# matthieugomez/LeastSquaresOptim.jl

Hardware: AMD Instinct MI355X
Metric: lm_lsmr_outer_iterations_per_sec (higher is better)
Workload: dtype f64

## Files before the change

leastsquaresoptim.jl_amd/csrc/lsq_lsmr.hip:

```cpp
#include <chrono>
#include <cmath>
#include <cstdlib>

#include "lsq_solver.h"
#include "lsq_spmv.h"

static constexpr int LSQ_LOOKAHEAD_DEFAULT = 2;

__device__ __forceinline__ void publish(LsqMailbox *mail, const LsmrState *st) {
    unsigned long long w = ((unsigned long long)(st->epoch & 0x7fffffu) << 41) |
                           ((unsigned long long)(st->done ? 1 : 0) << 40) |
                           ((unsigned long long)(st->istop & 0xff) << 32) | (unsigned)st->iter;
    __hip_atomic_store((unsigned long long *)mail, w, __ATOMIC_RELEASE, __HIP_MEMORY_SCOPE_SYSTEM);
}

__global__ void __launch_bounds__(LSQ_NT)
k_lsmr_prep(int n, const double *__restrict__ colsum, double *__restrict__ damp, double *__restrict__ P,
            double *__restrict__ dg, double *__restrict__ ux, int custom_p) {
    for (int j = blockIdx.x * LSQ_NT + threadIdx.x; j < n; j += gridDim.x * LSQ_NT) {
        double s = colsum[j];
        if (damp) {
            double d = damp[j];
            s += d;
            double r = sqrt(d);
// ... 335 lines not shown
#pragma unroll
    for (int k = 0; k < R; ++k) {
        const int i = tid + k * 1024;
        if (i < n) {
            acc += cs[k];
            double gi = gv[k];
            if (lm.lo && lm.x[i] <= lm.lo[i] && gi > 0.0) gi = 0.0;
            else if (lm.hi && lm.x[i] >= lm.hi[i] && gi < 0.0) gi = 0.0;
            double a = fabs(gi);
            if (isnan(a)) a = INFINITY;
            mg = fmax(mg, a);
        }
    }
    acc = wave_sum(acc);
    mg = wave_max(mg);
    if ((tid & 63) == 0) {
        sh[tid >> 6] = acc;
        shm[tid >> 6] = mg;
    }
    __syncthreads();
    if (tid == 0) {
        double tt = 0.0, tm = shm[0];
        for (int w = 0; w < 16; ++w) tt += sh[w];
        for (int w = 1; w < 16; ++w) tm = fmax(tm, shm[w]);
        s_mean = tt / n;
        if (blockIdx.x == 0) {
            *lm.out_grad = tm;
            st->iter = 0; st->istop = 0; st->done = 0; st->notdone = 1; st->first = 1;
            st->atol = atol; st->btol = btol; st->ctol = ctol;
            st->maxiter = maxiter; st->epoch = epoch; st->cu = 0.0;
            pu[0] = ysumsq;
            *npu = 1;
        }
    }
    __syncthreads();
    const double lo_d = lm.min_diag * s_mean, hi_d = lm.max_diag * s_mean;
    const double beta = dampened_norm(ysumsq, 0.0);
    const bool beta_zero = !(beta > 0.0);
    const double inv_beta = beta > 0.0 ? 1.0 / beta : 1.0;
    double a2 = 0.0;
    const int j = blockIdx.x * 1024 + tid;
    if (j < n) {
        double c0 = 0.0, g0 = 0.0;
#pragma unroll
        for (int k = 0; k < R; ++k)
            if (k == (int)blockIdx.x) { c0 = cs[k]; g0 = gv[k]; }
        double c = c0;
        c = c > hi_d ? hi_d : (c < lo_d ? lo_d : c);
        const double d = c * lm.inv_delta;
        const double s = c0 + d;
        const double r = sqrt(d);
        dg[j] = r;
        damp[j] = r;
        ux[j] = 0.0;
        const double Pj = s > 0.0 ? 1.0 / sqrt(s) : 0.0;
        P[j] = Pj;
        if (!beta_zero) {
            const double w = g0 * inv_beta * Pj;
            v[j] = w;
            if (wout) wout[j] = colscale ? (w * Pj) * colscale[j] : w * Pj;
            a2 = w * w;
        }
    }
    __syncthreads();
    const double bv = block_sum<1024>(a2, sh);
    if (tid == 0) {
        pv[blockIdx.x] = bv;
        if (blockIdx.x == 0) *npv = (int)gridDim.x;
    }
}

struct EpiBuf {
    static constexpr bool REDUCE = false;
    const int *done;
    int extra_blocks;
    double *out;
    double *partials;
    unsigned *counter;
    __device__ void seg(int j, double dot, double &) const { out[j] = dot; }
    __device__ void extra(int, double &) const {}
    __device__ void finalize(double) const {}
};
__global__ void __launch_bounds__(LSQ_NT) k_rowshard_sumsq(const double *pu, const int *npu, double *out, const int *done,
                                                            double *xbuf, int n) {
    if (done && *done) {
        for (int i = threadIdx.x; i <= n; i += LSQ_NT) xbuf[i] = 0.0;
        return;
    }
    double a, b, c2;
    ordered_sum256x3(pu, npu, nullptr, nullptr, nullptr, nullptr, a, b, c2);
    if (threadIdx.x == 0) *out = a;
}
extern "C" int lsq_solver_set_row_allreduce(lsq_solver *s, lsq_device_allreduce_callback cb, void *user, long long global_rows) {
    if (!s || s->kind != LSQ_LSMR) {
        lsq_set_error("row-sharded solves: LSMR() only");
        return LSQ_EARG;
    }
    s->row_cb = cb;
    s->row_user = user;
    s->global_rows = cb ? global_rows : 0;
    s->colsum_g_uid = 0;
    s->colsum_g_version = ~0ull;
    if (cb && !s->d_xbuf) {
        LSQ_HIP(hipMalloc(&s->d_xbuf, (size_t)(s->n + 2 + 256) * sizeof(double)));
        LSQ_ZERO(s->d_xbuf, 0, (size_t)(s->n + 2 + 256) * sizeof(double));
        LSQ_HIP(hipMalloc(&s->d_one, sizeof(int)));
        const int one = 1;
        LSQ_HIP(hipMemcpy(s->d_one, &one, sizeof(int), hipMemcpyHostToDevice));
    }
    return LSQ_OK;
}
int lsq_rowshard_colsum(lsq_solver *s, lsq_mat *J, const double **out) {
    const double *local = lsq_cached_colsum(J);
    if (!local) return LSQ_EHIP;
    *out = local;
    if (!s->row_cb) return LSQ_OK;
    lsq_ctx *c = s->ctx;
    if (!s->d_colsum_g) LSQ_HIP(hipMalloc(&s->d_colsum_g, (size_t)(s->n > 0 ? s->n : 1) * sizeof(double)));
    if (s->colsum_g_uid != J->uid || s->colsum_g_version != J->version) {
        LSQ_TRY(lsq_d2d(c, s->d_colsum_g, local, (size_t)J->n * sizeof(double)));
        if (s->row_cb(s->d_colsum_g, J->n, (void *)c->stream, s->row_user) != 0) {
            lsq_set_error("row all-reduce callback reported failure");
            return LSQ_ECALLBACK;
        }
        s->colsum_g_uid = J->uid;
        s->colsum_g_version = J->version;
    }
    *out = s->d_colsum_g;
    return LSQ_OK;
}
static int rowshard_adjoint(lsq_solver *s, lsq_mat *J, const double *src, EpiV ev, const double *pu, const int *npu) {
    lsq_ctx *c = s->ctx;
    const int n = J->n;
    EpiBuf eb{ev.done, 0, s->d_xbuf, nullptr, nullptr};
    LSQ_TRY(launch_product(J, 1, src, eb));
    LSQ_LAUNCH(k_rowshard_sumsq, dim3(1), dim3(LSQ_NT), 0, c->stream, pu, npu, s->d_xbuf + n, ev.done, s->d_xbuf, n);
    LSQ_HIP(hipGetLastError());
    if (s->row_cb(s->d_xbuf, n + 1, (void *)c->stream, s->row_user) != 0) {
        lsq_set_error("row all-reduce callback reported failure");
        return LSQ_ECALLBACK;
    }
    ev.pu = s->d_xbuf + n;
    ev.npu = s->d_one;
    const int nb = lsq_div_up(n, LSQ_CMB_COLS);
    LSQ_LAUNCH((k_combine<EpiV>), dim3(std::min(nb, 2048)), dim3(LSQ_NT), 0, c->stream, s->d_xbuf, n, 1, ev, nb);
    LSQ_HIP(hipGetLastError());
    return LSQ_OK;
}

int lsq_lsmr_alloc(lsq_solver *s) {
    size_t nb = (size_t)(s->n > 0 ? s->n : 1) * sizeof(double);
    LSQ_HIP(hipMalloc(&s->d_state, 2 * sizeof(LsmrState)));
    LSQ_ZERO(s->d_state, 0, 2 * sizeof(LsmrState));
    s->f3_elems = 4 * (size_t)(s->n > 0 ? s->n : 1) + 2 * 4096 + 8 + 16 + 8;
    LSQ_HIP(hipMalloc(&s->d_f3, s->f3_elems * sizeof(double)));
    LSQ_ZERO(s->d_f3, 0, s->f3_elems * sizeof(double));
    LSQ_HIP(hipMalloc(&s->d_u, (size_t)(s->m > 0 ? s->m : 1) * sizeof(double)));
    LSQ_HIP(hipMalloc(&s->d_ux, nb));
    LSQ_HIP(hipMalloc(&s->d_v, nb));
    LSQ_HIP(hipMalloc(&s->d_h, nb));
    LSQ_HIP(hipMalloc(&s->d_hbar, nb));
    LSQ_HIP(hipMalloc(&s->d_t, nb));
    LSQ_HIP(hipMalloc(&s->d_P, nb));
    LSQ_HIP(hipMalloc(&s->d_dg, nb));
    LSQ_HIP(hipMalloc(&s->d_rhs, nb));
    LSQ_HIP(hipMalloc(&s->d_red, 4 * 4096 * sizeof(double) + 64));
    LSQ_ZERO(s->d_red, 0, 4 * 4096 * sizeof(double) + 64);
    return LSQ_OK;
}

void lsq_lsmr_free(lsq_solver *s) {
    hipFree(s->d_state); hipFree(s->d_u); hipFree(s->d_ux); hipFree(s->d_v); hipFree(s->d_h);
    hipFree(s->d_hbar); hipFree(s->d_t); hipFree(s->d_P); hipFree(s->d_dg); hipFree(s->d_rhs); hipFree(s->d_red);
    hipFree(s->d_xbuf); hipFree(s->d_one); hipFree(s->d_colsum_g); hipFree(s->d_f3);
}

static inline int nvec_grid(const lsq_ctx *c, int n) {
    int g = lsq_div_up(n > 0 ? n : 1, LSQ_NT);
    int cap = c->num_cus * 4;
    return g > cap ? cap : g;
}

bool lsq_lsmr_takes_lm_prep(const lsq_solver *s, const lsq_mat *J) {
    return s->kind == LSQ_LSMR && J->n <= LSMR_LM_PREP_MAX_N && (s->row_cb || !lsq_small_mat(J)) && !s->precond_cb && !s->gen_ldiv &&
           !getenv("LSQ_LSMR_SEPARATE_SETUP");
}

struct LsmrProgress {
    bool ours, done;
    int istop, iter;
    LsmrProgress(unsigned long long w, unsigned epoch)
        : ours((unsigned)(w >> 41) == epoch), done(((w >> 40) & 1ull) != 0), istop((int)((w >> 32) & 0xff)), iter((int)(w & 0xffffffffu)) {}
};
static inline unsigned long long lsmr_progress_word(const lsq_ctx *c) { return *(volatile unsigned long long *)c->h_mail; }

struct StopPredictor {
    double t1_prev, t2_prev, ratio2;
    int hint_it;
    int update(const LsqMailbox *mail, unsigned long long w, int it, double atol, double btol) {
        if (!(it > hint_it && it >= 1)) return 0;
        const double h1 = mail->test1, h2 = mail->test2;
        const unsigned long long w2 = *(volatile unsigned long long *)mail;
        if (!(w2 == w && h1 > 0.0 && h2 > 0.0)) return 0;
        if (t2_prev > 0.0 && h2 < t2_prev) ratio2 = std::min(0.95, std::max(1e-4, h2 / t2_prev));
        int k = 1 << 20;
        if (h2 > atol && ratio2 < 1.0) k = std::min(k, (int)std::ceil(std::log(atol / h2) / std::log(ratio2) - 1e-9));
        if (t1_prev > 0.0 && h1 < 0.98 * t1_prev && h1 > btol)
            k = std::min(k, (int)std::ceil(std::log(btol / h1) / std::log(h1 / t1_prev) - 1e-9));
        t1_prev = h1; t2_prev = h2; hint_it = it;
        return k < (1 << 20) ? it + std::max(1, k) : 0;
    }
};

struct LsmrRun {
    int it = 0, istop = 0;
    bool finished = false;
    bool tail_ran = false;
    bool see(const LsmrProgress &p) {
        if (p.ours) it = p.iter;
        if (p.ours && p.done) { istop = p.istop; finished = true; }
        return finished;
    }
};

static int lsmr_stream_drained(lsq_ctx *c, unsigned epoch, int committed, const LsmrState *d_st, bool spent, LsmrRun &r) {
    const hipError_t sq = hipStreamQuery(c->stream);
    if (sq != hipSuccess && sq != hipErrorNotReady) {
        lsq_set_error("HIP error inside the LSMR iteration: %s", hipGetErrorString(sq));
        return LSQ_EHIP;
    }
    if (sq != hipSuccess) return LSQ_OK;
    const LsmrProgress p(lsmr_progress_word(c), epoch);
    if (p.ours && (p.done || p.iter >= committed)) return LSQ_OK;
    LsmrState hs;
    LSQ_HIP(hipMemcpy(&hs, d_st, sizeof(hs), hipMemcpyDeviceToHost));
    r.it = hs.iter;
    if (hs.done) {
        r.istop = hs.istop;
        r.finished = true;
    } else if (spent) {
        lsq_set_error("lsmr: iteration budget exhausted without a stop rule");
        return LSQ_EHIP;
    }
    return LSQ_OK;
}

struct LsmrProf {
    size_t base[2];
    std::vector<int> iter[2];
};
static void lsmr_drop_idle_samples(lsq_ctx *c, LsmrProf &p, int it) {
    for (int k = 0; k < 2; ++k) {
        auto &v = c->prof_ev[k];
        while (v.size() > p.base[k] && !p.iter[k].empty() && p.iter[k].back() > it) {
            hipEventDestroy(v.back()); v.pop_back();
            hipEventDestroy(v.back()); v.pop_back();
            p.iter[k].pop_back();
        }
    }
}

struct LsmrWork {
    lsq_solver *s;
    lsq_ctx *c;
    lsq_mat *J;
    const double *d_y;
    double *d_x;
    int m, n;
    bool damped, sharded;
    bool fused;
    double atol, btol, conlim;
    int maxiter, lookahead;
    unsigned epoch;
    int gn;
    const double *dgk;
    const LsmrTail *tail;
    bool dynamic, spec;
    LsmrState *stb[2];
    double *pu, *pv;
    int *npu, *npv;
    double *pxb[2];
    int *npxb[2];
    double *vset;
    double *fx[2], *fhbar[2], *fh[2];
    double *fw;
    double *fpu[2];
    int *fnpu;
    LsmrHandoff *fho;
};

static EpiV lsmr_epi_v(const LsmrWork &W) {
    return EpiV{&W.stb[0]->done, 0, W.stb[0], W.pu, W.npu, nullptr, nullptr, W.s->d_P, W.dgk, nullptr, W.s->d_v, W.pv, W.npv,
                nullptr, 0.0, 0.0, 0, 0};
}
static void lsmr_launch_update(const LsmrWork &W, bool summed, const double *px_in, const int *npx_in, int out) {
    lsq_solver *s = W.s; lsq_ctx *c = W.c;
    LSQ_LAUNCH(k_lsmr_update, dim3(W.gn), dim3(LSQ_NT), 0, c->stream, W.n, W.stb[0], c->d_mail,
                       summed ? (const double *)(s->d_xbuf + W.n) : (const double *)W.pu,
                       summed ? (const int *)s->d_one : (const int *)W.npu, W.pv, W.npv, px_in, npx_in, W.pxb[out], W.npxb[out],
                       W.dgk, s->d_ux, s->d_P, s->d_v, s->d_h, s->d_hbar, s->d_rhs, W.d_x, s->d_t, c->d_partials, lsq_ctr(c, 3));
}

static int lsmr_enqueue_setup(const LsmrWork &W, double *d_damp, const double *d_Jty, double y_sumsq, const LsmrLmPrep *lm,
                              const double *colsum, int custom_p) {
    lsq_solver *s = W.s; lsq_ctx *c = W.c; lsq_mat *J = W.J;
    const int m = W.m, n = W.n;
    LsmrState *st = W.stb[0];
// ... 122 lines not shown
        }
        if (!(wait_at > 0 && r.it < wait_at)) {
            if (k1 == enq + 1) {
                LSQ_TRY(launch_k2());
                spins = 0;
                continue;
            }
            if (enq - r.it < W.lookahead + 1 && enq < W.maxiter + 1) {
                const bool guess = W.spec && planned > 0 && enq >= planned && enq >= 1;
                const bool unknown = W.spec && enq == 1 && pred.hint_it == 0 && tail->predict <= 3;
                LSQ_TRY(launch_k1(guess || unknown));
                if (guess || unknown) {
                    wait_at = enq;
                    wait_is_guess = guess;
                }
                spins = 0;
                continue;
            }
        }
        if (c->idle_hook) lsq_run_idle_hook(c);
        if ((++spins & 0x3ffu) != 0) continue;
        LSQ_TRY(lsmr_stream_drained(c, W.epoch, k1 - 1, W.stb[k1 & 1], enq >= W.maxiter + 1, r));
    }
    lsmr_drop_idle_samples(c, prof, r.it);
    if (r.istop == 99) {
        lsq_set_error("lsmr: the in-launch hand-off of k_lsmr_fused timed out");
        return LSQ_EHIP;
    }
    if (wait_at > 0 && wait_is_guess) c->tail_spec[0]++;
    return LSQ_OK;
}

static int lsmr_run_four(const LsmrWork &W, StopPredictor &pred, LsmrRun &r) {
    lsq_solver *s = W.s; lsq_ctx *c = W.c; lsq_mat *J = W.J;
    const LsmrTail *tail = W.tail;
    const bool sharded = W.sharded;
    const int maxiter = W.maxiter;
    LsmrState *st = W.stb[0];
    EpiU eu{&st->done, 0, st, W.d_y, s->d_u, W.n, s->d_dg, s->d_t, s->d_ux, W.pu, W.npu, nullptr, 0.0};
    EpiV ev = lsmr_epi_v(W);
    ev.ux = W.damped ? s->d_ux : nullptr;
    int planned = W.spec ? tail->predict : 0;
    int tail_at = 0;
    int enq = 0;
    LsmrProf prof{{c->prof_ev[0].size(), c->prof_ev[1].size()}, {}};
    unsigned long long spins = 0;
    while (!r.finished) {
        const unsigned long long w = lsmr_progress_word(c);
        const LsmrProgress p(w, W.epoch);
        if (r.see(p)) break;
        if (W.spec && p.ours && tail_at > 0 && r.it >= tail_at) {
            c->tail_spec[0]++;
            c->tail_spec[1]++;
            tail_at = 0;
            planned = 0;
        }
        if (W.dynamic && p.ours) {
            const int stop = pred.update(c->h_mail, w, r.it, W.atol, W.btol);
            if (stop > 0 && tail_at == 0) planned = stop;
        }
        if (W.spec && tail_at == 0 && planned > 0 && enq >= planned && enq > r.it) {
            LSQ_TRY(tail->fn(&st->notdone, tail->user));
            tail_at = enq;
        }
        const bool hold = tail_at > 0 && enq == tail_at && r.it < tail_at;
        const bool want = sharded ? (p.ours && enq == r.it && enq < maxiter) : (!hold && enq - r.it < W.lookahead && enq < maxiter);
        if (want) {
            const int chunk = sharded ? (int)std::min<long long>(W.lookahead, (long long)maxiter - enq) : 1;
            for (int q = 0; q < chunk; ++q) {
                if (c->prof_kernels & 1) lsq_prof_mark(c, 0, 0);
                {
                    const size_t before = c->prof_ev[0].size();
                    LSQ_TRY(launch_product(J, 0, s->d_t, eu));
                    if (c->prof_ev[0].size() > before) prof.iter[0].push_back(enq + 1);
                }
                if (c->prof_kernels & 1) lsq_prof_mark(c, 0, 1);
                eu.uold = s->d_u;
                const int cur = enq & 1;
                ev.px = W.damped ? W.pxb[cur] : nullptr;
                ev.npx = W.npxb[cur];
                if (c->prof_kernels & 2) lsq_prof_mark(c, 1, 0);
                {
                    const size_t before = c->prof_ev[1].size();
                    if (sharded) LSQ_TRY(rowshard_adjoint(s, J, s->d_u, ev, W.pu, W.npu));
                    else LSQ_TRY(launch_product(J, 1, s->d_u, ev));
                    if (c->prof_ev[1].size() > before) prof.iter[1].push_back(enq + 1);
                }
                if (c->prof_kernels & 2) lsq_prof_mark(c, 1, 1);
                lsmr_launch_update(W, sharded, ev.px, ev.npx, cur ^ 1);
                LSQ_HIP(hipGetLastError());
                ++enq;
            }
            spins = 0;
            continue;
        }
        if (c->idle_hook) lsq_run_idle_hook(c);
        if ((++spins & 0x3ffu) != 0) continue;
        LSQ_TRY(lsmr_stream_drained(c, W.epoch, enq, st, enq >= maxiter, r));
    }
    lsmr_drop_idle_samples(c, prof, r.it);
    if (tail_at > 0) {
        c->tail_spec[0]++;
        if (r.it > tail_at) c->tail_spec[1]++;
        else r.tail_ran = true;
    }
    return LSQ_OK;
}

int lsq_lsmr_solve(lsq_solver *s, lsq_mat *J, const double *d_y, double *d_damp, double *d_x, int *nmul,
                   const double *d_Jty, double y_sumsq, const LsmrLmPrep *lm, const LsmrTail *tail) {
    lsq_ctx *c = s->ctx;
    const int m = J->m, n = J->n;
    if (m != s->m || n != s->n) {
        lsq_set_error("lsmr: solver allocated for %dx%d, Jacobian is %dx%d", s->m, s->n, m, n);
        return LSQ_EDIM;
    }
    if (s->gen_ldiv) {
        if (s->row_cb) {
            lsq_set_error("row-sharded solves take diagonal preconditioners only");
            return LSQ_EARG;
        }
        LSQ_TRY(lsq_lsmr_general_solve(s, J, d_y, d_damp, d_x, nmul));
        s->last_lsmr_path = 4;
        return tail && tail->fn ? tail->fn(nullptr, tail->user) : LSQ_OK;
    }
    const bool sharded = s->row_cb != nullptr;
    if (lsq_small_mat(J) && !s->precond_cb && !sharded) {
        LSQ_TRY(lsq_lsmr_exact_solve(s, J, d_y, d_damp, d_x, nmul));
        s->last_lsmr_path = 1;
        return tail && tail->fn ? tail->fn(nullptr, tail->user) : LSQ_OK;
    }
    LsmrWork W;
    W.s = s; W.c = c; W.J = J; W.d_y = d_y; W.d_x = d_x; W.m = m; W.n = n;
    W.damped = d_damp != nullptr; W.sharded = sharded;
    W.atol = 1e-6; W.btol = W.damped ? 0.5 : 1e-6; W.conlim = 1e8;
    const long long rows = (sharded ? s->global_rows : (long long)m) + (W.damped ? n : 0);
    W.maxiter = (int)std::max<long long>(rows, n);
    W.lookahead = lsq_dbg_serial ? 1 : LSQ_LOOKAHEAD_DEFAULT;
    W.epoch = (++c->mail_epoch) & 0x7fffffu;
    if (J->kind == LSQ_MAT_CSC) LSQ_TRY(lsq_ensure_csr(J));
    const bool four_env = getenv("LSQ_LSMR_FOUR_LAUNCHES") != nullptr;
    W.fused = !four_env && !sharded && J->kind == LSQ_MAT_CSC && J->srows.active && J->srows.ncw == 1 && J->scols.active &&
              n >= 1 && m >= 1 && c->num_cus >= 8;
    W.gn = nvec_grid(c, n); W.dgk = W.damped ? s->d_dg : nullptr;
    W.tail = tail;
    W.dynamic = tail && tail->fn && tail->dynamic && !sharded;
    W.spec = tail && tail->fn && !sharded && (tail->predict > 0 || W.dynamic);
    W.stb[0] = s->d_state; W.stb[1] = s->d_state + 1;
    W.pv = s->d_red + 4096;
    W.pxb[0] = s->d_red + 2 * 4096; W.pxb[1] = s->d_red + 3 * 4096;
    int *const counts = (int *)(s->d_red + 4 * 4096);
    W.npv = counts + 1; W.npxb[0] = counts + 2; W.npxb[1] = counts + 3;
    double *const f3 = s->d_f3;
    W.fx[0] = s->d_rhs; W.fx[1] = f3; W.fhbar[0] = s->d_hbar; W.fhbar[1] = f3 + n; W.fh[0] = s->d_h; W.fh[1] = f3 + 2 * (size_t)n;
    W.fw = f3 + 3 * (size_t)n;
    W.fpu[0] = f3 + 4 * (size_t)n; W.fpu[1] = W.fpu[0] + 4096;
    W.fnpu = (int *)(W.fpu[1] + 4096); W.fho = (LsmrHandoff *)(W.fpu[1] + 4096 + 8);
    W.vset = W.fused ? s->d_t : s->d_v;
    W.pu = W.fused ? W.fpu[0] : s->d_red;
    W.npu = W.fused ? W.fnpu : counts;
    const double *colsum = nullptr;
    LSQ_TRY(lsq_rowshard_colsum(s, J, &colsum));
    const int custom_p = s->precond_cb ? 1 : 0;
    if (custom_p) {
        LSQ_HIP(hipStreamSynchronize(c->stream));
        if (s->precond_cb(s->d_P, J, d_damp, s->precond_user) != 0) {
            lsq_set_error("preconditioner callback reported failure");
            return LSQ_ECALLBACK;
        }
    }
    *(volatile unsigned long long *)c->h_mail = 0ull;
    LSQ_TRY(lsmr_enqueue_setup(W, d_damp, d_Jty, y_sumsq, lm, colsum, custom_p));

    StopPredictor pred{-1.0, -1.0, s->lsmr_ratio2, 0};
    LsmrRun r;
    LSQ_TRY(W.fused ? lsmr_run_fused(W, pred, r) : lsmr_run_four(W, pred, r));
    s->last_iter = r.it;
    s->last_istop = r.istop;
    s->last_lsmr_path = W.fused ? 3 : 2;
    if (nmul) *nmul = 2 * r.it;
    if (W.dynamic && pred.t2_prev > 0.0) s->lsmr_ratio2 = pred.ratio2;
    if (tail && tail->fn && !r.tail_ran) LSQ_TRY(tail->fn(nullptr, tail->user));
    return LSQ_OK;
}
```

leastsquaresoptim.jl_amd/csrc/lsq_lsmr3.h:

```cpp
#pragma once

constexpr int LSQ_FUSED_UB_MAX = 4;
struct LsmrHandoff {
    unsigned long long w[8];
};
__device__ __forceinline__ void lsmr_handoff_write(LsmrHandoff *ho, unsigned tag, double vs, double cu, int done) {
    const unsigned long long t = (unsigned long long)tag << 32;
    const unsigned long long bv = (unsigned long long)__double_as_longlong(vs), bc = (unsigned long long)__double_as_longlong(cu);
    __hip_atomic_store(&ho->w[0], t | (bv & 0xffffffffull), __ATOMIC_RELAXED, __HIP_MEMORY_SCOPE_AGENT);
    __hip_atomic_store(&ho->w[1], t | (bv >> 32), __ATOMIC_RELAXED, __HIP_MEMORY_SCOPE_AGENT);
    __hip_atomic_store(&ho->w[2], t | (bc & 0xffffffffull), __ATOMIC_RELAXED, __HIP_MEMORY_SCOPE_AGENT);
    __hip_atomic_store(&ho->w[3], t | (bc >> 32), __ATOMIC_RELAXED, __HIP_MEMORY_SCOPE_AGENT);
    __hip_atomic_store(&ho->w[4], t | (unsigned)done, __ATOMIC_RELAXED, __HIP_MEMORY_SCOPE_AGENT);
}
__device__ __forceinline__ void lsmr_handoff_fail(LsmrHandoff *ho, unsigned tag) {
    __hip_atomic_store(&ho->w[6], (unsigned long long)tag, __ATOMIC_RELAXED, __HIP_MEMORY_SCOPE_AGENT);
}
struct LsmrHandoffWords { unsigned long long w[5]; };
__device__ __forceinline__ LsmrHandoffWords lsmr_handoff_request(const LsmrHandoff *ho) {
    LsmrHandoffWords r;
#pragma unroll
    for (int k = 0; k < 5; ++k) r.w[k] = __hip_atomic_load(&ho->w[k], __ATOMIC_RELAXED, __HIP_MEMORY_SCOPE_AGENT);
    return r;
}
__device__ __forceinline__ bool lsmr_handoff_valid(const LsmrHandoffWords &r, unsigned tag) {
    bool ok = true;
#pragma unroll
    for (int k = 0; k < 5; ++k) ok = ok && (unsigned)(r.w[k] >> 32) == tag;
    return ok;
}
struct LsmrFused {
    const LsmrState *st_in;
    LsmrState *st_out;
    LsqMailbox *mail;
    LsmrHandoff *ho;
    unsigned tag;
    unsigned tag_prev;
    const double *pu_in; const int *npu_in;
    double *pu_out; int *npu_out;
    const double *px_in; const int *npx_in;
    double *px_out; int *npx_out;
    const double *pv; const int *npv;
    const double *vt;
    const double *w;
    const double *P, *dg;
    const double *h_in, *hbar_in, *x_in;
    double *h_out, *hbar_out, *x_out;
    double *v, *xout, *ux;
    const double *uold; double *unew;
    int n, ub;
    int test_no_record;
    int cautious;
};

__device__ inline void lsmr_decide(LsmrState &s, double total) {
    s.iter += 1;
    s.normx = sqrt(total);
    const double test1 = s.normr / s.normb;
    const double test2 = s.normAr / (s.normA * s.normr);
    const double test3 = 1.0 / s.condA;
    const double t1 = test1 / (1.0 + s.normA * s.normx / s.normb);
    const double rtol = s.btol + s.atol * s.normA * s.normx / s.normb;
    int istop = 0;
    if (s.iter >= s.maxiter) istop = 7;
    else if (1.0 + test3 <= 1.0) istop = 6;
    else if (1.0 + test2 <= 1.0) istop = 5;
    else if (1.0 + t1 <= 1.0) istop = 4;
    else if (test3 <= s.ctol) istop = 3;
    else if (test2 <= s.atol) istop = 2;
    else if (test1 <= rtol) istop = 1;
    s.istop = istop;
    if (istop) { s.done = 1; s.notdone = 0; }
}

constexpr long long LSQ_FUSED_SPIN_LIMIT = 1LL << 24;

__device__ __forceinline__ void publish_relaxed(LsqMailbox *mail, const LsmrState *st) {
    unsigned long long w = ((unsigned long long)(st->epoch & 0x7fffffu) << 41) |
                           ((unsigned long long)(st->done ? 1 : 0) << 40) |
                           ((unsigned long long)(st->istop & 0xff) << 32) | (unsigned)st->iter;
    __hip_atomic_store((unsigned long long *)mail, w, __ATOMIC_RELAXED, __HIP_MEMORY_SCOPE_SYSTEM);
}

__device__ __forceinline__ void ordered_sum512x3(const double *pa, const int *na, const double *pb, const int *nb,
                                                 const double *pc, const int *nc, double &ra, double &rb, double &rc) {
    __shared__ double s_w5[3][4];
    __shared__ double s_tot5[3];
    const int tid = threadIdx.x;
    if (tid < 256) {
        const double a0 = pa ? pa[tid] : 0.0, b0 = pb ? pb[tid] : 0.0, c0 = pc ? pc[tid] : 0.0;
        const double a1 = pa ? pa[tid + 256] : 0.0, b1 = pb ? pb[tid + 256] : 0.0, c1 = pc ? pc[tid + 256] : 0.0;
        const int ca = pa ? *na : 0, cb = pb ? *nb : 0, cc = pc ? *nc : 0;
        double a = tid < ca ? a0 : 0.0, b = tid < cb ? b0 : 0.0, c = tid < cc ? c0 : 0.0;
        if (tid + 256 < ca) a += a1;
        if (tid + 256 < cb) b += b1;
        if (tid + 256 < cc) c += c1;
        for (int i = tid + 512; i < ca; i += 256) a += pa[i];
        for (int i = tid + 512; i < cb; i += 256) b += pb[i];
        for (int i = tid + 512; i < cc; i += 256) c += pc[i];
        a = wave_sum(a);
        b = wave_sum(b);
        c = wave_sum(c);
        if ((tid & 63) == 0) {
            s_w5[0][tid >> 6] = a;
            s_w5[1][tid >> 6] = b;
            s_w5[2][tid >> 6] = c;
        }
    }
    __syncthreads();
    if (tid < 3) s_tot5[tid] = ((s_w5[tid][0] + s_w5[tid][1]) + s_w5[tid][2]) + s_w5[tid][3];
    __syncthreads();
    ra = s_tot5[0];
    rb = s_tot5[1];
    rc = s_tot5[2];
    __syncthreads();
}

__device__ __forceinline__ void lsq_lds_barrier() { asm volatile("s_waitcnt lgkmcnt(0)\n\ts_barrier" ::: "memory"); }
template <bool IS_MAX>
__device__ __forceinline__ double lsq_block_reduce_lds(double v, double *sh ) {
    v = IS_MAX ? wave_max(v) : wave_sum(v);
    const int lane = threadIdx.x & 63, w = threadIdx.x >> 6;
    if (lane == 0) sh[w] = v;
    lsq_lds_barrier();
    double r = 0.0;
    if (threadIdx.x == 0) {
        r = sh[0];
#pragma unroll
        for (int i = 1; i < LSQ_BIG_NT / 64; ++i) r = IS_MAX ? fmax(r, sh[i]) : r + sh[i];
    }
    lsq_lds_barrier();
    return r;
}

template <int = 0>
__global__ void __launch_bounds__(LSQ_BIG_NT) k_lsmr_fused(SellDev S, int wrows, int m, int nxpad, LsmrFused a) {
    extern __shared__ __attribute__((aligned(16))) double smem[];
    __shared__ double sh[LSQ_BIG_NT / 64];
    __shared__ LsmrState ns;
    __shared__ double s_vs, s_cu;
    __shared__ int s_done;
    double *xl = smem;
    double *yw = smem + nxpad;
    const int tid = threadIdx.x, lane = tid & 63, wv = tid >> 6;
    const int n = a.n;
    const bool upd = (int)blockIdx.x < a.ub;

    if (upd) {
        static_assert(sizeof(LsmrState) % 8 == 0 && sizeof(LsmrState) / 8 <= LSQ_BIG_NT, "state copy: one 8-byte word per thread");
        constexpr int NQ = (LSQ_LDS_X_MAX + LSQ_BIG_NT - 1) / LSQ_BIG_NT;
        double xi[NQ], hbi[NQ], hi[NQ];
#pragma unroll
        for (int q = 0; q < NQ; ++q) {
            const int j = min(tid + q * LSQ_BIG_NT, n - 1);
            xi[q] = a.x_in[j];
            hbi[q] = a.hbar_in[j];
            hi[q] = a.h_in[j];
        }
        if (tid < (int)(sizeof(LsmrState) / 8)) ((unsigned long long *)&ns)[tid] = ((const unsigned long long *)a.st_in)[tid];
        const bool prev_failed = a.tag_prev != 0u &&
                                 (unsigned)__hip_atomic_load(&a.ho->w[6], __ATOMIC_RELAXED, __HIP_MEMORY_SCOPE_AGENT) == a.tag_prev;
        double beta2, betax2, alpha2;
        ordered_sum512x3(a.pu_in, a.npu_in, a.px_in, a.npx_in, a.pv, a.npv, beta2, betax2, alpha2);
        if (ns.done) {
            if (blockIdx.x == 0) {
                if (tid < (int)(sizeof(LsmrState) / 8)) ((unsigned long long *)a.st_out)[tid] = ((const unsigned long long *)&ns)[tid];
                if (tid == 0) {
                    lsmr_handoff_write(a.ho, a.tag, 1.0, 0.0, 1);
                    publish_relaxed(a.mail, &ns);
                }
            }
            return;
        }
        const bool was_first = ns.first != 0;
        if (tid == 0) lsmr_scalars(ns, beta2, betax2, alpha2, a.dg != nullptr, a.px_in != nullptr);
        __syncthreads();
        if (!was_first) {
            const double c1 = ns.c1, c2 = ns.c2;
            double acc = 0.0;
#pragma unroll
            for (int q = 0; q < NQ; ++q) {
                const double hb = hbi[q] * c1 + hi[q];
                const double xj = xi[q] + c2 * hb;
                acc += (tid + q * LSQ_BIG_NT < n) ? xj * xj : 0.0;
            }
            const double total = block_sum<LSQ_BIG_NT>(acc, sh);
            if (tid == 0) lsmr_decide(ns, total);
        } else if (tid == 0) {
            ns.first = 0;
            if (!(ns.normAr != 0.0)) { ns.done = 1; ns.notdone = 0; }
        }
        if (tid == 0 && prev_failed) { ns.istop = 99; ns.done = 1; ns.notdone = 0; }
        __syncthreads();
        const bool done_now = ns.done != 0;
        const double vs = ns.vscale, cu = ns.cu, c1 = ns.c1, c2 = ns.c2, c3 = ns.c3;
        if (blockIdx.x == 0) {
            if (tid == 0 && !a.test_no_record) lsmr_handoff_write(a.ho, a.tag, vs, cu, done_now ? 1 : 0);
            if (tid < (int)(sizeof(LsmrState) / 8)) ((unsigned long long *)a.st_out)[tid] = ((const unsigned long long *)&ns)[tid];
            if (tid == 0) {
                if (!was_first) {
                    __hip_atomic_store((double *)&a.mail->test1, ns.normr / ns.normb, __ATOMIC_RELAXED, __HIP_MEMORY_SCOPE_SYSTEM);
                    __hip_atomic_store((double *)&a.mail->test2, ns.normAr / (ns.normA * ns.normr), __ATOMIC_RELAXED, __HIP_MEMORY_SCOPE_SYSTEM);
                }
                publish_relaxed(a.mail, &ns);
            }
        }
        constexpr int NU = (NQ + 2) / 3;
        double e_vt[NU], e_P[NU], e_dg[NU], e_ux[NU], e_h[NU], e_hb[NU], e_x[NU];
#pragma unroll
        for (int k = 0; k < NU; ++k) {
            const int j = min((int)(blockIdx.x + k * a.ub) * LSQ_BIG_NT + tid, n - 1);
            e_vt[k] = a.vt[j];
            e_P[k] = a.P ? a.P[j] : 1.0;
            e_dg[k] = a.dg ? a.dg[j] : 0.0;
            e_ux[k] = a.dg ? a.ux[j] : 0.0;
            e_h[k] = a.h_in[j];
            e_hb[k] = a.hbar_in[j];
            e_x[k] = a.x_in[j];
        }
        double aux = 0.0;
#pragma unroll
        for (int k = 0; k < NU; ++k) {
            const int j = (int)(blockIdx.x + k * a.ub) * LSQ_BIG_NT + tid;
            if (j >= n) continue;
            const double Pj = e_P[k];
            const double vj = e_vt[k] * vs;
            a.v[j] = vj;
            if (was_first) {
                a.h_out[j] = vj;
                a.hbar_out[j] = 0.0;
                a.x_out[j] = 0.0;
                a.xout[j] = 0.0;
            } else {
                const double hj = e_h[k];
                const double hb = e_hb[k] * c1 + hj;
                a.hbar_out[j] = hb;
                const double xj = e_x[k] + c2 * hb;
                a.x_out[j] = xj;
                a.h_out[j] = hj * c3 + vj;
                a.xout[j] = a.P ? xj * Pj : xj;
            }
            if (a.dg && !done_now) {
                const double tj = a.P ? vj * Pj : vj;
                const double un = tj * e_dg[k] - cu * e_ux[k];
                a.ux[j] = un;
                aux += un * un;
            }
        }
        if (done_now) return;
        const double bux = lsq_block_reduce_lds<false>(aux, sh);
        if (tid == 0) {
            a.px_out[blockIdx.x] = bux;
            if (blockIdx.x == 0) *a.npx_out = a.ub;
        }
        return;
    }

    constexpr int XR = (LSQ_LDS_X_MAX + LSQ_BIG_NT - 1) / LSQ_BIG_NT;
    {
        double xr[XR];
#pragma unroll
        for (int q = 0; q < XR; ++q) xr[q] = a.w[min(tid + q * LSQ_BIG_NT, n - 1)];
        const int dflag = a.st_in->done;
#pragma unroll
        for (int q = 0; q < XR; ++q)
            if (tid + q * LSQ_BIG_NT < n) xl[tid + q * LSQ_BIG_NT] = xr[q];
        if (dflag) return;
    }
    constexpr int Q = LSQ_SELL_ROWS_MAX / LSQ_BIG_NT;
    const int pb = (int)blockIdx.x - a.ub, npb = (int)gridDim.x - a.ub;
    double racc = 0.0;
    bool have_scalars = false;
    if (a.cautious) {
        if (tid == 0) {
            LsmrHandoffWords rec = lsmr_handoff_request(a.ho);
            long long spins = 0;
            while (!lsmr_handoff_valid(rec, a.tag)) {
                if (++spins > (a.test_no_record ? 4096 : LSQ_FUSED_SPIN_LIMIT)) break;
                __builtin_amdgcn_s_sleep(8);
                rec = lsmr_handoff_request(a.ho);
            }
            const bool ok = spins <= (a.test_no_record ? 4096 : LSQ_FUSED_SPIN_LIMIT);
            s_vs = __longlong_as_double((long long)((rec.w[0] & 0xffffffffull) | (rec.w[1] << 32)));
            s_cu = __longlong_as_double((long long)((rec.w[2] & 0xffffffffull) | (rec.w[3] << 32)));
            s_done = ok ? (int)(rec.w[4] & 0xffffffffull) : 2;
            if (!ok) lsmr_handoff_fail(a.ho, a.tag);
        }
        __syncthreads();
        if (s_done) return;
        have_scalars = true;
    }
    for (int w = pb; w < S.nblocks; w += npb) {
        const int base = w * wrows, rows = min(wrows, m - base);
        const int s0 = w * S.spw, s1 = s0 + S.spw;
        double pre[Q];
#pragma unroll
        for (int q = 0; q < Q; ++q) pre[q] = a.uold[base + min(tid + q * LSQ_BIG_NT, rows - 1)];
        LsmrHandoffWords rec;
#pragma unroll
        for (int k = 0; k < 5; ++k) rec.w[k] = 0ull;
        {
            constexpr int NW = LSQ_BIG_NT / 64;
            int sidx = s0 + wv;
            SellSliceRef A = sell_slice_ref(S, sidx, s1, lane);
            __syncthreads();
            unsigned long long poll = 0ull;
            for (; sidx < s1; sidx += NW) {
                if (!have_scalars && (unsigned)(poll >> 32) == a.tag && (poll & 1ull)) break;
                if (!have_scalars) poll = __hip_atomic_load(&a.ho->w[4], __ATOMIC_RELAXED, __HIP_MEMORY_SCOPE_AGENT);
                const SellSliceRef r = A;
                A = sell_slice_ref(S, sidx + NW, s1, lane);
                if (!have_scalars && tid == 0 && sidx + NW >= s1) rec = lsmr_handoff_request(a.ho);
                const size_t oa = (size_t)r.sm.x + lane * 2;
                const unsigned pos = r.inf & LSQ_SELL_POS_MASK;
                double sum = 0.0, sq = 0.0;
                sell_lane_sum<false>(S.val + oa, S.idx16 + oa, r.sm.y, (int)(r.inf >> LSQ_SELL_POS_BITS), xl, sum, sq, lane);
                if (pos != LSQ_SELL_POS_MASK) yw[pos] = sum;
            }
        }
        if (!have_scalars && tid == 0) {
            long long spins = 0;
            while (!lsmr_handoff_valid(rec, a.tag)) {
                if (++spins > (a.test_no_record ? 4096 : LSQ_FUSED_SPIN_LIMIT)) break;
                __builtin_amdgcn_s_sleep(8);
                rec = lsmr_handoff_request(a.ho);
            }
            const bool ok = spins <= (a.test_no_record ? 4096 : LSQ_FUSED_SPIN_LIMIT);
            s_vs = __longlong_as_double((long long)((rec.w[0] & 0xffffffffull) | (rec.w[1] << 32)));
            s_cu = __longlong_as_double((long long)((rec.w[2] & 0xffffffffull) | (rec.w[3] << 32)));
            s_done = ok ? (int)(rec.w[4] & 0xffffffffull) : 2;
            if (!ok) lsmr_handoff_fail(a.ho, a.tag);
        }
        have_scalars = true;
        __syncthreads();
        if (s_done) return;
        const double vs = s_vs, cu = s_cu;
#pragma unroll
        for (int q = 0; q < Q; ++q) {
            const int i = tid + q * LSQ_BIG_NT;
            if (i < rows) {
                const double un = vs * yw[i] - cu * pre[q];
                a.unew[base + i] = un;
                racc += un * un;
            }
        }
    }
    const double bv = block_sum<LSQ_BIG_NT>(racc, sh);
    if (tid == 0) {
        a.pu_out[pb] = bv;
        if (pb == 0) *a.npu_out = npb;
    }
}
```

Measured before the change: 4210.

## Stage fused LSMR kernel vectors into LDS via async DMA and prefetch first slice

After: 4201. Within noise of the previous version (-0.2%).

```diff
diff --git a/leastsquaresoptim.jl_amd/csrc/lsq_lsmr.hip b/leastsquaresoptim.jl_amd/csrc/lsq_lsmr.hip
--- a/leastsquaresoptim.jl_amd/csrc/lsq_lsmr.hip
+++ b/leastsquaresoptim.jl_amd/csrc/lsq_lsmr.hip
@@ -511,7 +511,7 @@
     size_t nb = (size_t)(s->n > 0 ? s->n : 1) * sizeof(double);
     LSQ_HIP(hipMalloc(&s->d_state, 2 * sizeof(LsmrState)));
     LSQ_ZERO(s->d_state, 0, 2 * sizeof(LsmrState));
-    s->f3_elems = 4 * (size_t)(s->n > 0 ? s->n : 1) + 2 * 4096 + 8 + 16 + 8;
+    s->f3_elems = 4 * (((size_t)(s->n > 0 ? s->n : 1) + 1) & ~(size_t)1) + 2 * 4096 + 8 + 16 + 8;
     LSQ_HIP(hipMalloc(&s->d_f3, s->f3_elems * sizeof(double)));
     LSQ_ZERO(s->d_f3, 0, s->f3_elems * sizeof(double));
     LSQ_HIP(hipMalloc(&s->d_u, (size_t)(s->m > 0 ? s->m : 1) * sizeof(double)));
@@ -940,9 +940,10 @@
     int *const counts = (int *)(s->d_red + 4 * 4096);
     W.npv = counts + 1; W.npxb[0] = counts + 2; W.npxb[1] = counts + 3;
     double *const f3 = s->d_f3;
-    W.fx[0] = s->d_rhs; W.fx[1] = f3; W.fhbar[0] = s->d_hbar; W.fhbar[1] = f3 + n; W.fh[0] = s->d_h; W.fh[1] = f3 + 2 * (size_t)n;
-    W.fw = f3 + 3 * (size_t)n;
-    W.fpu[0] = f3 + 4 * (size_t)n; W.fpu[1] = W.fpu[0] + 4096;
+    const size_t np2 = ((size_t)n + 1) & ~(size_t)1;
+    W.fx[0] = s->d_rhs; W.fx[1] = f3; W.fhbar[0] = s->d_hbar; W.fhbar[1] = f3 + np2; W.fh[0] = s->d_h; W.fh[1] = f3 + 2 * np2;
+    W.fw = f3 + 3 * np2;
+    W.fpu[0] = f3 + 4 * np2; W.fpu[1] = W.fpu[0] + 4096;
     W.fnpu = (int *)(W.fpu[1] + 4096); W.fho = (LsmrHandoff *)(W.fpu[1] + 4096 + 8);
     W.vset = W.fused ? s->d_t : s->d_v;
     W.pu = W.fused ? W.fpu[0] : s->d_red;
diff --git a/leastsquaresoptim.jl_amd/csrc/lsq_lsmr3.h b/leastsquaresoptim.jl_amd/csrc/lsq_lsmr3.h
--- a/leastsquaresoptim.jl_amd/csrc/lsq_lsmr3.h
+++ b/leastsquaresoptim.jl_amd/csrc/lsq_lsmr3.h
@@ -149,19 +149,31 @@
     if (upd) {
         static_assert(sizeof(LsmrState) % 8 == 0 && sizeof(LsmrState) / 8 <= LSQ_BIG_NT, "state copy: one 8-byte word per thread");
         constexpr int NQ = (LSQ_LDS_X_MAX + LSQ_BIG_NT - 1) / LSQ_BIG_NT;
-        double xi[NQ], hbi[NQ], hi[NQ];
+        constexpr int NU = (NQ + 2) / 3;
+        const SellStageTail xtail = sell_stage_dma<(NQ + 1) / 2>(a.x_in, smem, n, tid);
+        double hbi[NQ], hi[NQ];
 #pragma unroll
         for (int q = 0; q < NQ; ++q) {
             const int j = min(tid + q * LSQ_BIG_NT, n - 1);
-            xi[q] = a.x_in[j];
             hbi[q] = a.hbar_in[j];
             hi[q] = a.h_in[j];
+        }
+        double e_vt[NU], e_P[NU], e_dg[NU], e_ux[NU];
+#pragma unroll
+        for (int k = 0; k < NU; ++k) {
+            const int j = min((int)(blockIdx.x + k * a.ub) * LSQ_BIG_NT + tid, n - 1);
+            e_vt[k] = a.vt[j];
+            e_P[k] = a.P ? a.P[j] : 1.0;
+            e_dg[k] = a.dg ? a.dg[j] : 0.0;
+            e_ux[k] = a.dg ? a.ux[j] : 0.0;
         }
         if (tid < (int)(sizeof(LsmrState) / 8)) ((unsigned long long *)&ns)[tid] = ((const unsigned long long *)a.st_in)[tid];
         const bool prev_failed = a.tag_prev != 0u &&
                                  (unsigned)__hip_atomic_load(&a.ho->w[6], __ATOMIC_RELAXED, __HIP_MEMORY_SCOPE_AGENT) == a.tag_prev;
         double beta2, betax2, alpha2;
         ordered_sum512x3(a.pu_in, a.npu_in, a.px_in, a.npx_in, a.pv, a.npv, beta2, betax2, alpha2);
+        sell_stage_tail_write(xtail, smem);
+        sell_stage_wait();
         if (ns.done) {
             if (blockIdx.x == 0) {
                 if (tid < (int)(sizeof(LsmrState) / 8)) ((unsigned long long *)a.st_out)[tid] = ((const unsigned long long *)&ns)[tid];
@@ -173,7 +185,22 @@
             return;
         }
         const bool was_first = ns.first != 0;
-        if (tid == 0) lsmr_scalars(ns, beta2, betax2, alpha2, a.dg != nullptr, a.px_in != nullptr);
+        if (wv == 0) {
+            double *park = smem + nxpad + lane;
+#pragma unroll
+            for (int q = 0; q < NQ; ++q) {
+                park[(2 * q) * 64] = hbi[q];
+                park[(2 * q + 1) * 64] = hi[q];
+            }
+            asm volatile("" ::: "memory");
+            if (tid == 0) lsmr_scalars(ns, beta2, betax2, alpha2, a.dg != nullptr, a.px_in != nullptr);
+            asm volatile("" ::: "memory");
+#pragma unroll
+            for (int q = 0; q < NQ; ++q) {
+                hbi[q] = park[(2 * q) * 64];
+                hi[q] = park[(2 * q + 1) * 64];
+            }
+        }
         __syncthreads();
         if (!was_first) {
             const double c1 = ns.c1, c2 = ns.c2;
@@ -181,7 +208,7 @@
 #pragma unroll
             for (int q = 0; q < NQ; ++q) {
                 const double hb = hbi[q] * c1 + hi[q];
-                const double xj = xi[q] + c2 * hb;
+                const double xj = smem[min(tid + q * LSQ_BIG_NT, n - 1)] + c2 * hb;
                 acc += (tid + q * LSQ_BIG_NT < n) ? xj * xj : 0.0;
             }
             const double total = block_sum<LSQ_BIG_NT>(acc, sh);
@@ -205,24 +232,22 @@
                 publish_relaxed(a.mail, &ns);
             }
         }
-        constexpr int NU = (NQ + 2) / 3;
-        double e_vt[NU], e_P[NU], e_dg[NU], e_ux[NU], e_h[NU], e_hb[NU], e_x[NU];
+        double aux = 0.0;
+        int ubs = a.ub, bxs = (int)blockIdx.x;
+        asm volatile("" : "+s"(ubs), "+s"(bxs));
 #pragma unroll
         for (int k = 0; k < NU; ++k) {
-            const int j = min((int)(blockIdx.x + k * a.ub) * LSQ_BIG_NT + tid, n - 1);
-            e_vt[k] = a.vt[j];
-            e_P[k] = a.P ? a.P[j] : 1.0;
-            e_dg[k] = a.dg ? a.dg[j] : 0.0;
-            e_ux[k] = a.dg ? a.ux[j] : 0.0;
-            e_h[k] = a.h_in[j];
-            e_hb[k] = a.hbar_in[j];
-            e_x[k] = a.x_in[j];
-        }
-        double aux = 0.0;
-#pragma unroll
-        for (int k = 0; k < NU; ++k) {
-            const int j = (int)(blockIdx.x + k * a.ub) * LSQ_BIG_NT + tid;
+            const int g = bxs + k * ubs;
+            const int j = g * LSQ_BIG_NT + tid;
             if (j >= n) continue;
+            double e_h = 0.0, e_hb = 0.0;
+#pragma unroll
+            for (int q = 0; q < NQ; ++q)
+                if (q == g) {
+                    e_h = hi[q];
+                    e_hb = hbi[q];
+                }
+            const double e_x = smem[j];
             const double Pj = e_P[k];
             const double vj = e_vt[k] * vs;
             a.v[j] = vj;
@@ -232,10 +257,10 @@
                 a.x_out[j] = 0.0;
                 a.xout[j] = 0.0;
             } else {
-                const double hj = e_h[k];
-                const double hb = e_hb[k] * c1 + hj;
+                const double hj = e_h;
+                const double hb = e_hb * c1 + hj;
                 a.hbar_out[j] = hb;
-                const double xj = e_x[k] + c2 * hb;
+                const double xj = e_x + c2 * hb;
                 a.x_out[j] = xj;
                 a.h_out[j] = hj * c3 + vj;
                 a.xout[j] = a.P ? xj * Pj : xj;
@@ -256,19 +281,13 @@
         return;
     }
 
-    constexpr int XR = (LSQ_LDS_X_MAX + LSQ_BIG_NT - 1) / LSQ_BIG_NT;
-    {
-        double xr[XR];
-#pragma unroll
-        for (int q = 0; q < XR; ++q) xr[q] = a.w[min(tid + q * LSQ_BIG_NT, n - 1)];
-        const int dflag = a.st_in->done;
-#pragma unroll
-        for (int q = 0; q < XR; ++q)
-            if (tid + q * LSQ_BIG_NT < n) xl[tid + q * LSQ_BIG_NT] = xr[q];
-        if (dflag) return;
-    }
-    constexpr int Q = LSQ_SELL_ROWS_MAX / LSQ_BIG_NT;
+    constexpr int NW = LSQ_BIG_NT / 64;
     const int pb = (int)blockIdx.x - a.ub, npb = (int)gridDim.x - a.ub;
+    const bool hasblk = pb < S.nblocks;
+    const int sA = pb * S.spw + wv, sE = hasblk ? (pb + 1) * S.spw : 0;
+    int2 smA = make_int2(0, 0), smB = make_int2(0, 0);
+    if (sA < sE) smA = S.smeta[__builtin_amdgcn_readfirstlane(sA)];
+    if (sA + NW < sE) smB = S.smeta[__builtin_amdgcn_readfirstlane(sA + NW)];
     double racc = 0.0;
     bool have_scalars = false;
     if (a.cautious) {
@@ -290,59 +309,113 @@
         if (s_done) return;
         have_scalars = true;
     }
-    for (int w = pb; w < S.nblocks; w += npb) {
-        const int base = w * wrows, rows = min(wrows, m - base);
-        const int s0 = w * S.spw, s1 = s0 + S.spw;
-        double pre[Q];
+    constexpr int XR = (LSQ_LDS_X_MAX + LSQ_BIG_NT - 1) / LSQ_BIG_NT;
+    constexpr int Q = LSQ_SELL_ROWS_MAX / LSQ_BIG_NT;
+    SellSliceRef ref0, ref1;
+    ref0.sm = smA; ref0.inf = LSQ_SELL_POS_MASK;
+    ref1.sm = smB; ref1.inf = LSQ_SELL_POS_MASK;
+    if (sA < sE) ref0.inf = S.info[(size_t)sA * 64 + lane];
+    if (sA + NW < sE) ref1.inf = S.info[(size_t)(sA + NW) * 64 + lane];
+    const SellStageTail wtail = sell_stage_dma<(XR + 1) / 2>(a.w, xl, n, tid);
+    const int dflag = a.st_in->done;
+    double pre[Q];
+    if (hasblk) {
+        const int base = pb * wrows, rows = min(wrows, m - base);
 #pragma unroll
         for (int q = 0; q < Q; ++q) pre[q] = a.uold[base + min(tid + q * LSQ_BIG_NT, rows - 1)];
-        LsmrHandoffWords rec;
-#pragma unroll
-        for (int k = 0; k < 5; ++k) rec.w[k] = 0ull;
-        {
-            constexpr int NW = LSQ_BIG_NT / 64;
-            int sidx = s0 + wv;
-            SellSliceRef A = sell_slice_ref(S, sidx, s1, lane);
+    }
+    const int2 sm0 = make_int2(__builtin_amdgcn_readfirstlane(ref0.sm.x), __builtin_amdgcn_readfirstlane(ref0.sm.y));
+    const bool head = sA < sE;
+    SellHead H;
+    if (head) sell_head_load(H, S.val, S.idx16, sm0.x, sm0.y, lane);
+    sell_stage_tail_write(wtail, xl);
+    sell_stage_wait();
+    __syncthreads();
+    {
+        int d = dflag;
+        asm volatile("" : "+v"(d));
+        if (d) return;
+    }
+    LsmrHandoffWords rec;
+#pragma unroll
+    for (int k = 0; k < 5; ++k) rec.w[k] = 0ull;
+    unsigned long long poll = 0ull;
+    int sidx = pb * S.spw + wv;
+    SellSliceRef A;
+    A.sm = make_int2(0, 0);
+    A.inf = LSQ_SELL_POS_MASK;
+    if (hasblk) {
+        if (head) {
+            const int s1 = (pb + 1) * S.spw;
+            if (!have_scalars) poll = __hip_atomic_load(&a.ho->w[4], __ATOMIC_RELAXED, __HIP_MEMORY_SCOPE_AGENT);
+            unsigned inf0 = ref0.inf;
+            asm volatile("" : "+v"(inf0));
+            A = ref1;
+            asm volatile("" : "+v"(A.sm.x), "+v"(A.sm.y), "+v"(A.inf));
+            if (!have_scalars && tid == 0 && sidx + NW >= s1) rec = lsmr_handoff_request(a.ho);
+            const size_t oa = (size_t)sm0.x + lane * 2;
+            const unsigned pos = inf0 & LSQ_SELL_POS_MASK;
+            double sum = 0.0, sq = 0.0;
+            sell_lane_sum_head<false>(H, S.val + oa, S.idx16 + oa, sm0.y, (int)(inf0 >> LSQ_SELL_POS_BITS), xl, sum, sq, lane);
+            if (pos != LSQ_SELL_POS_MASK) yw[pos] = sum;
+            sidx += NW;
+        }
+        for (int w = pb;;) {
+            const int base = w * wrows, rows = min(wrows, m - base);
+            const int s0 = w * S.spw, s1 = s0 + S.spw;
+            if (w != pb) {
+#pragma unroll
+                for (int q = 0; q < Q; ++q) pre[q] = a.uold[base + min(tid + q * LSQ_BIG_NT, rows - 1)];
+#pragma unroll
+                for (int k = 0; k < 5; ++k) rec.w[k] = 0ull;
+                poll = 0ull;
+                sidx = s0 + wv;
+                A = sell_slice_ref(S, sidx, s1, lane);
+                __syncthreads();
+            }
+            {
+                for (; sidx < s1; sidx += NW) {
+                    if (!have_scalars && (unsigned)(poll >> 32) == a.tag && (poll & 1ull)) break;
+                    if (!have_scalars) poll = __hip_atomic_load(&a.ho->w[4], __ATOMIC_RELAXED, __HIP_MEMORY_SCOPE_AGENT);
+                    const SellSliceRef r = A;
+                    A = sell_slice_ref(S, sidx + NW, s1, lane);
+                    if (!have_scalars && tid == 0 && sidx + NW >= s1) rec = lsmr_handoff_request(a.ho);
+                    const size_t oa = (size_t)r.sm.x + lane * 2;
+                    const unsigned pos = r.inf & LSQ_SELL_POS_MASK;
+                    double sum = 0.0, sq = 0.0;
+                    sell_lane_sum<false>(S.val + oa, S.idx16 + oa, r.sm.y, (int)(r.inf >> LSQ_SELL_POS_BITS), xl, sum, sq, lane);
+                    if (pos != LSQ_SELL_POS_MASK) yw[pos] = sum;
+                }
+            }
+            if (!have_scalars && tid == 0) {
+                long long spins = 0;
+                while (!lsmr_handoff_valid(rec, a.tag)) {
+                    if (++spins > (a.test_no_record ? 4096 : LSQ_FUSED_SPIN_LIMIT)) break;
+                    __builtin_amdgcn_s_sleep(8);
+                    rec = lsmr_handoff_request(a.ho);
+                }
+                const bool ok = spins <= (a.test_no_record ? 4096 : LSQ_FUSED_SPIN_LIMIT);
+                s_vs = __longlong_as_double((long long)((rec.w[0] & 0xffffffffull) | (rec.w[1] << 32)));
+                s_cu = __longlong_as_double((long long)((rec.w[2] & 0xffffffffull) | (rec.w[3] << 32)));
+                s_done = ok ? (int)(rec.w[4] & 0xffffffffull) : 2;
+                if (!ok) lsmr_handoff_fail(a.ho, a.tag);
+            }
+            have_scalars = true;
             __syncthreads();
-            unsigned long long poll = 0ull;
-            for (; sidx < s1; sidx += NW) {
-                if (!have_scalars && (unsigned)(poll >> 32) == a.tag && (poll & 1ull)) break;
-                if (!have_scalars) poll = __hip_atomic_load(&a.ho->w[4], __ATOMIC_RELAXED, __HIP_MEMORY_SCOPE_AGENT);
-                const SellSliceRef r = A;
-                A = sell_slice_ref(S, sidx + NW, s1, lane);
-                if (!have_scalars && tid == 0 && sidx + NW >= s1) rec = lsmr_handoff_request(a.ho);
-                const size_t oa = (size_t)r.sm.x + lane * 2;
-                const unsigned pos = r.inf & LSQ_SELL_POS_MASK;
-                double sum = 0.0, sq = 0.0;
-                sell_lane_sum<false>(S.val + oa, S.idx16 + oa, r.sm.y, (int)(r.inf >> LSQ_SELL_POS_BITS), xl, sum, sq, lane);
-                if (pos != LSQ_SELL_POS_MASK) yw[pos] = sum;
-            }
-        }
-        if (!have_scalars && tid == 0) {
-            long long spins = 0;
-            while (!lsmr_handoff_valid(rec, a.tag)) {
-                if (++spins > (a.test_no_record ? 4096 : LSQ_FUSED_SPIN_LIMIT)) break;
-                __builtin_amdgcn_s_sleep(8);
-                rec = lsmr_handoff_request(a.ho);
-            }
-            const bool ok = spins <= (a.test_no_record ? 4096 : LSQ_FUSED_SPIN_LIMIT);
-            s_vs = __longlong_as_double((long long)((rec.w[0] & 0xffffffffull) | (rec.w[1] << 32)));
-            s_cu = __longlong_as_double((long long)((rec.w[2] & 0xffffffffull) | (rec.w[3] << 32)));
-            s_done = ok ? (int)(rec.w[4] & 0xffffffffull) : 2;
-            if (!ok) lsmr_handoff_fail(a.ho, a.tag);
-        }
-        have_scalars = true;
-        __syncthreads();
-        if (s_done) return;
-        const double vs = s_vs, cu = s_cu;
-#pragma unroll
-        for (int q = 0; q < Q; ++q) {
-            const int i = tid + q * LSQ_BIG_NT;
-            if (i < rows) {
-                const double un = vs * yw[i] - cu * pre[q];
-                a.unew[base + i] = un;
-                racc += un * un;
-            }
+            sell_stage_wait();
+            if (s_done) return;
+            const double vs = s_vs, cu = s_cu;
+#pragma unroll
+            for (int q = 0; q < Q; ++q) {
+                const int i = tid + q * LSQ_BIG_NT;
+                if (i < rows) {
+                    const double un = vs * yw[i] - cu * pre[q];
+                    a.unew[base + i] = un;
+                    racc += un * un;
+                }
+            }
+            w += npb;
+            if (w >= S.nblocks) break;
         }
     }
     const double bv = block_sum<LSQ_BIG_NT>(racc, sh);
```
